# fmfi-compbio/warpstr

Measured on NVIDIA B200. Metric: caller_reads_per_s, higher is better.
Workload: dtype f64

## Files before the change

### warpstr_b200/csrc/dtw.cu

```cuda
#include "wstr_internal.h"

namespace {

constexpr int CH = WSTR_SIG_CHUNK;
constexpr unsigned FULL = 0xffffffffu;

__device__ __forceinline__ uint32_t smem_u32(const void *p) {
    return static_cast<uint32_t>(__cvta_generic_to_shared(p));
}
__device__ __forceinline__ void mbar_init(uint64_t *bar, int count) {
    asm volatile("mbarrier.init.shared::cta.b64 [%0], %1;" ::"r"(smem_u32(bar)), "r"(count) : "memory");
}
__device__ __forceinline__ void fence_barrier_init() {
    asm volatile("fence.mbarrier_init.release.cluster;" ::: "memory");
    asm volatile("fence.proxy.async.shared::cta;" ::: "memory");
}
__device__ __forceinline__ void bulk_load(void *dst, const void *src, uint32_t bytes, uint64_t *bar) {
    asm volatile("mbarrier.arrive.expect_tx.shared::cta.b64 _, [%0], %1;" ::"r"(smem_u32(bar)), "r"(bytes)
                 : "memory");
    asm volatile(
        "cp.async.bulk.shared::cluster.global.mbarrier::complete_tx::bytes [%0], [%1], %2, [%3];" ::"r"(
            smem_u32(dst)),
        "l"(src), "r"(bytes), "r"(smem_u32(bar))
        : "memory");
}
__device__ __forceinline__ bool mbar_try_wait(uint64_t *bar, uint32_t parity) {
    uint32_t ok;
    asm volatile(
        "{\n"
        ".reg .pred p;\n"
        "mbarrier.try_wait.parity.shared::cta.b64 p, [%1], %2;\n"
        "selp.u32 %0, 1, 0, p;\n"
        "}\n"
        : "=r"(ok)
        : "r"(smem_u32(bar)), "r"(parity)
        : "memory");
    return ok != 0;
}

__device__ __forceinline__ double dinf() { return __longlong_as_double(0x7ff0000000000000LL); }

template <int K, int MV>
struct LaneState {
    double v[K];
    double D[K];
    double R[MV - 1][K];
};

template <int MV>
__host__ __device__ constexpr int role_reg(int m, int ph) {
    return ((m - 1 - ph) % (MV - 1) + (MV - 1)) % (MV - 1);
}

template <int K, int MV, bool SHORT, int PH>
__device__ __forceinline__ double offer(const LaneState<K, MV> &s, int k) {
    if (SHORT) {
        if (MV >= 3) return s.R[role_reg<MV>(MV >= 3 ? MV - 2 : 1, PH)][k];
        return s.D[k];
    }
    return s.R[role_reg<MV>(MV - 1, PH)][k];
}

template <int K, int MV, int PH>
__device__ __forceinline__ void advance(LaneState<K, MV> &s, int k, double ae, double stay) {
#pragma unroll
    for (int m = MV - 2; m >= 1; --m) s.R[role_reg<MV>(m, PH)][k] += ae;
    s.R[role_reg<MV>(MV - 1, PH)][k] = stay;
}

template <int KG>
struct LaneConsts {
    uint32_t band_bits;
    uint32_t src0;
    uint32_t gsrc[KG];
};

template <int KG>
__host__ __device__ constexpr int q_row_len() { return 32 * KG + 40; }

template <int DEG>
struct DegOf {
    static constexpr bool LOW = DEG >= 100 && DEG < 200;
    static constexpr bool GRADED = DEG >= 200;
    static constexpr int MAX = GRADED ? (DEG - 200) / 10 : (LOW ? DEG - 100 : DEG);
};
template <int KG, int DEG>
__host__ __device__ constexpr int slot_deg(int g) {
    if (DegOf<DEG>::GRADED) return g == KG - 1 ? (DEG - 200) / 10 : (g == KG - 2 ? (DEG - 200) % 10 : 1);
    return (DegOf<DEG>::LOW && g < KG - 1) ? 1 : DegOf<DEG>::MAX;
}
template <int KC, int KG, int DEG>
__host__ __device__ constexpr int slot_bit(int g) {
    int b = KC;
    for (int i = 0; i < g; ++i) b += slot_deg<KG, DEG>(i);
    return b;
}
template <int KC, int KG, int DEG>
struct DirFmt {
    static constexpr int NB = slot_bit<KC, KG, DEG>(KG - 1) + DegOf<DEG>::MAX;
    static constexpr int RPW = 32 / NB;
    static_assert(NB <= 32 && RPW >= 1, "direction codes of one row must fit a 32-bit word");
};

struct DirOut {
    uint32_t acc;
    int sh;
    uint32_t *ptr;
};

__device__ __forceinline__ double take_min(const double best, uint32_t &codes, const double cand, const uint32_t bit) {
    double out;
    asm("{\n"
        ".reg .pred p;\n"
        "setp.lt.f64 p, %2, %3;\n"
        "selp.f64 %0, %2, %3, p;\n"
        "@p or.b32 %1, %1, %4;\n"
        "}\n"
        : "=d"(out), "+r"(codes)
        : "d"(cand), "d"(best), "r"(bit));
    return out;
}

template <int KC, int KG, int DEG, int MV, bool SHORT, bool BAND, int PH, int SUB>
__device__ __forceinline__ void dp_row(LaneState<KC + KG, MV> &s, const LaneConsts<KG> &lc, const double x,
                                       double *__restrict__ Qpub, const double *__restrict__ Qrow, DirOut &o) {
    constexpr int K = KC + KG;
    constexpr int NB = DirFmt<KC, KG, DEG>::NB, RPW = DirFmt<KC, KG, DEG>::RPW;
    constexpr int B0 = SUB >= 0 ? SUB * NB : 0;
    const double INF = dinf();

#pragma unroll
    for (int g = 0; g < KG; ++g) Qpub[g * 32] = offer<K, MV, SHORT, PH>(s, KC + g);
    Qpub[KG * 32] = offer<K, MV, SHORT, PH>(s, KC - 1);
    __syncwarp();

    uint32_t codes = SUB >= 0 ? o.acc : 0u;

    const double qfirst = *reinterpret_cast<const double *>(reinterpret_cast<const unsigned char *>(Qrow) + lc.src0);
#pragma unroll
    for (int k = KC - 1; k >= 0; --k) {
        const double ae = fabs(x - s.v[k]);
        const double qprev = k > 0 ? offer<K, MV, SHORT, PH>(s, k > 0 ? k - 1 : 0) : qfirst;
        const double stay = s.D[k] + ae;
        double best = stay;
        best = take_min(best, codes, qprev + ae, 1u << (B0 + k));
        if (BAND) {
            if ((lc.band_bits >> k) & 1u) {
                best = INF;
                codes &= ~(1u << (B0 + k));
            }
        }
        advance<K, MV, PH>(s, k, ae, stay);
        s.D[k] = best;
    }

#pragma unroll
    for (int g = 0; g < KG; ++g) {
        const int k = KC + g;
        const double ae = fabs(x - s.v[k]);
        const double stay = s.D[k] + ae;
        double best = stay;
#pragma unroll
        for (int r = 0; r < DegOf<DEG>::MAX; ++r) {
            if (r < slot_deg<KG, DEG>(g)) {
                const uint32_t idx = (lc.gsrc[g] >> (8 * r)) & 0xffu;
                best = take_min(best, codes, Qrow[idx] + ae, 1u << (B0 + slot_bit<KC, KG, DEG>(g) + r));
            }
        }
        if (BAND) {
            if ((lc.band_bits >> k) & 1u) {
                best = INF;
                codes &= ~(((1u << slot_deg<KG, DEG>(g)) - 1u) << (B0 + slot_bit<KC, KG, DEG>(g)));
            }
        }
        advance<K, MV, PH>(s, k, ae, stay);
        s.D[k] = best;
    }

    if (SUB >= 0) {
        if (SUB == RPW - 1) {
            *o.ptr = codes;
            o.ptr += 32;
            o.acc = 0u;
        } else {
            o.acc = codes;
        }
    } else {
        o.acc |= codes << o.sh;
        o.sh += NB;
        if (o.sh > 32 - NB) {
            *o.ptr = o.acc;
            o.ptr += 32;
            o.acc = 0u;
            o.sh = 0;
        }
    }
}

template <int KC, int KG, int DEG, int MV, bool SHORT, bool BAND, bool ALIGNED, int PH = 0>
__device__ __forceinline__ void dp_rows_cycle(LaneState<KC + KG, MV> &s, const LaneConsts<KG> &lc,
                                              double (&xv)[MV - 1], const double *__restrict__ xnext,
                                              double *__restrict__ Qlane, const double *__restrict__ Qbase,
                                              DirOut &o) {
    constexpr int QL = q_row_len<KG>();
    constexpr int RPW = DirFmt<KC, KG, DEG>::RPW;
    constexpr int SUB = RPW == 1 ? 0 : (ALIGNED ? PH : -1);
    dp_row<KC, KG, DEG, MV, SHORT, BAND, PH, SUB>(s, lc, xv[PH], Qlane + PH * QL, Qbase + PH * QL, o);
    xv[PH] = xnext[PH];
    if constexpr (PH + 1 < MV - 1)
        dp_rows_cycle<KC, KG, DEG, MV, SHORT, BAND, ALIGNED, PH + 1>(s, lc, xv, xnext, Qlane, Qbase, o);
}

template <int KC, int KG, int DEG, int MV, bool SHORT, bool BAND>
__device__ __forceinline__ void dp_row_single(LaneState<KC + KG, MV> &s, const LaneConsts<KG> &lc, const double x,
                                              double *__restrict__ Qlane, const double *__restrict__ Qbase,
                                              DirOut &o) {
    constexpr int K = KC + KG;
    constexpr int SUB = DirFmt<KC, KG, DEG>::RPW == 1 ? 0 : -1;
    dp_row<KC, KG, DEG, MV, SHORT, BAND, 0, SUB>(s, lc, x, Qlane, Qbase, o);
    __syncwarp();
#pragma unroll
    for (int k = 0; k < K; ++k) {
        const double last = s.R[MV - 2][k];
#pragma unroll
        for (int m = MV - 2; m >= 1; --m) s.R[m][k] = s.R[m - 1][k];
        s.R[0][k] = last;
    }
}

template <int KC, int KG, int DEG, int MV, bool SHORT, bool BAND>
__device__ __forceinline__ void dp_segment(LaneState<KC + KG, MV> &s, const LaneConsts<KG> &lc,
                                           const double *__restrict__ xs, const int tile0, int i0, const int i1,
                                           double *__restrict__ Qlane, const double *__restrict__ Qbase, DirOut &o) {
    constexpr int CY = MV - 1;
    constexpr int RPW = DirFmt<KC, KG, DEG>::RPW;
    constexpr bool ALIGNED = RPW == CY && RPW > 1;
    const double *xp = xs + (i0 - tile0);
    if (ALIGNED) {
#pragma unroll 1
        for (; i0 < i1 && o.sh != 0; ++i0) {
            dp_row_single<KC, KG, DEG, MV, SHORT, BAND>(s, lc, *xp, Qlane, Qbase, o);
            xp += 1;
        }
    }
    double xv[CY];
#pragma unroll
    for (int j = 0; j < CY; ++j) xv[j] = xp[j];
#pragma unroll 1
    for (; i0 + CY <= i1; i0 += CY) {
        dp_rows_cycle<KC, KG, DEG, MV, SHORT, BAND, ALIGNED>(s, lc, xv, xp + CY, Qlane, Qbase, o);
        xp += CY;
    }
#pragma unroll 1
    for (; i0 < i1; ++i0) {
        dp_row_single<KC, KG, DEG, MV, SHORT, BAND>(s, lc, *xp, Qlane, Qbase, o);
        xp += 1;
    }
}

__device__ __forceinline__ int mask_run_end(const uint32_t *__restrict__ mw, int a, const int limit, uint32_t &bit) {
    uint32_t word = __ldg(mw + (a >> 5));
    bit = (word >> (a & 31)) & 1u;
    uint32_t diff = (bit ? ~word : word) >> (a & 31);
    int b = a;
    for (;;) {
        if (diff) {
            b += __ffs(diff) - 1;
            break;
        }
        b = (b | 31) + 1;
        if (b >= limit) break;
        word = __ldg(mw + (b >> 5));
        diff = bit ? ~word : word;
    }
    return b < limit ? b : limit;
}

template <int KC, int KG, int DEG, int MV, bool BAND, bool MASKED>
__device__ __forceinline__ void dp_tile_rows(LaneState<KC + KG, MV> &s, const LaneConsts<KG> &lc,
                                             const double *__restrict__ xs, const int tile0, int i0, const int i1,
                                             const uint32_t *__restrict__ mw_ptr, double *__restrict__ Qlane,
                                             const double *__restrict__ Qbase, DirOut &o) {
    if (!MASKED || !mw_ptr) {
        dp_segment<KC, KG, DEG, MV, false, BAND>(s, lc, xs, tile0, i0, i1, Qlane, Qbase, o);
        return;
    }
    while (i0 < i1) {
        uint32_t bit;
        const int b = mask_run_end(mw_ptr, i0, i1, bit);
        if (bit) dp_segment<KC, KG, DEG, MV, true, BAND>(s, lc, xs, tile0, i0, b, Qlane, Qbase, o);
        else dp_segment<KC, KG, DEG, MV, false, BAND>(s, lc, xs, tile0, i0, b, Qlane, Qbase, o);
        i0 = b;
    }
}

template <int RPW>
struct TbGeom {
    static constexpr int WRW = RPW == 1 ? 16 : 32 / RPW;
    static constexpr int ROWS = WRW * RPW;
    static constexpr int NBUF = 5;
    static constexpr int WORDS = NBUF * WRW * 32;
};

__device__ __forceinline__ void mbar_expect_tx(uint64_t *bar, uint32_t bytes) {
    asm volatile("mbarrier.arrive.expect_tx.shared::cta.b64 _, [%0], %1;" ::"r"(smem_u32(bar)), "r"(bytes)
                 : "memory");
}
template <int KC, int KG, int DEG>
__device__ __forceinline__ void traceback_warp(const DevAutomaton *A, const int T, const uint32_t *dir,
                                               const uint32_t *mw, int32_t *tr, int32_t *status_slot,
                                               const int lane, uint32_t *win, uint64_t *bar, uint32_t &phase_bits,
                                               const int32_t *spred) {
    constexpr int K = KC + KG;
    constexpr int NB = DirFmt<KC, KG, DEG>::NB, RPW = DirFmt<KC, KG, DEG>::RPW;
    using G = TbGeom<RPW>;
    constexpr int WRW = G::WRW, ROWS = G::ROWS, NBUF = G::NBUF;
    const int mv = A->mv;
    const int wtop = (T - 1) / RPW;
    const int wmin = mv / RPW;
    const int nwin = wtop / WRW + 1;

    auto issue = [&](int c) {
        if (lane != 0) return;
        const int b = c % NBUF;
        const int wh = wtop - c * WRW;
        const int wfirst = wh - WRW + 1;
        const int w0 = wfirst > wmin ? wfirst : wmin;
        const int n = wh - w0 + 1;
        if (n > 0)
            bulk_load(win + (b * WRW + (w0 - wfirst)) * 32, dir + static_cast<int64_t>(w0) * 32,
                      static_cast<uint32_t>(n) * 128u, &bar[b]);
        else
            mbar_expect_tx(&bar[b], 0u);
    };

    int i = T - 1;
    int pos = A->end_pos;
    int st = __ldg(A->state_of_pos + pos);
    bool failed = false;
    for (int c = 0; c < nwin && c < NBUF; ++c) issue(c);

    for (int c = 0; c < nwin; ++c) {
        const int b = c % NBUF;
        while (!mbar_try_wait(&bar[b], (phase_bits >> b) & 1u)) {
        }
        phase_bits ^= 1u << b;
        const int wh = wtop - c * WRW;
        const int hi = wh * RPW + RPW - 1;
        const int lo = hi - ROWS + 1 > 0 ? hi - ROWS + 1 : 0;
        if (i >= lo && i > 0 && !failed) {
            const int row = hi - lane;
            const bool mine = lane < ROWS && row >= lo && row <= i;
            const bool coded = mine && row >= mv;
            uint32_t mb = 0u;
            if (mw && mine) mb = (__ldg(mw + (row >> 5)) >> (row & 31)) & 1u;
            const int wr = mine ? row / RPW : wh;
            const uint32_t *wslot = win + (b * WRW + (wr - (wh - WRW + 1))) * 32;
            const int fsh = (row - wr * RPW) * NB;
            int my = st;
            for (;;) {
                const int hl = pos / K;
                const int u = pos - hl * K;
                uint32_t nib = 0u;
                if (coded && row <= i) {
                    const uint32_t f = wslot[hl] >> fsh;
                    if (u < KC) {
                        nib = (f >> u) & 1u;
                    } else {
                        const int g = u - KC;
                        int off = KC, width = 1;
#pragma unroll
                        for (int gg = 0; gg < KG; ++gg)
                            if (g == gg) {
                                off = slot_bit<KC, KG, DEG>(gg);
                                width = slot_deg<KG, DEG>(gg);
                            }
                        nib = (f >> off) & ((1u << width) - 1u);
                    }
                }
                const uint32_t moves = __ballot_sync(FULL, nib != 0u);
                if (moves == 0u) {
                    i = lo - 1;
                    break;
                }
                const int tm = __ffs(moves) - 1;
                const int rm = hi - tm;
                const uint32_t nibm = __shfl_sync(FULL, nib, tm);
                const int back = mv - static_cast<int>(__shfl_sync(FULL, mb, tm));
                const int code = 31 - __clz(nibm);
                const int32_t pp = spred[pos * DegOf<DEG>::MAX + code];
                if (rm < back || pp < 0) {
                    failed = true;
                    break;
                }
                const int pst = pp >> 16;
                if (row < rm) my = pst;
                if (rm - back + 1 < lo) {
                    const int r = lo - 1 - lane;
                    if (lane < back - 1 && r > rm - back) tr[r] = pst;
                }
                i = rm - back;
                pos = pp & 0xffff;
                st = pst;
                if (i < lo || i <= 0) break;
            }
            if (mine) tr[row] = my;
        }
        __syncwarp();
        if (c + NBUF < nwin) issue(c + NBUF);
    }
    if (lane == 0) {
        if (failed) *status_slot = WSTR_READ_BACKTRACK;
        else tr[0] = st;
    }
}

template <int KC, int KG, int DEG, int MV>
struct alignas(16) FillSmem {
    using G = TbGeom<DirFmt<KC, KG, DEG>::RPW>;
    double sig[2][CH];
    double Q[MV - 1][q_row_len<KG>()];
    uint32_t win[G::WORDS];
    int32_t pred[(KC + KG) * 32 * DegOf<DEG>::MAX];
    uint64_t bar[2];
    uint64_t tbar[G::NBUF];
};

#ifndef WSTR_K8_WARPS
#define WSTR_K8_WARPS 16
#endif
#ifdef WSTR_MAXNREG
#define WSTR_FILL_BOUNDS __maxnreg__(WSTR_MAXNREG)
#else
#define WSTR_FILL_BOUNDS                         \
    __launch_bounds__(32 * WSTR_WARPS_PER_CTA,   \
                      ((KC + KG) * (MV + 1) <= 45 && KG <= 1 && !MASKED ? WSTR_K8_WARPS                                          \
                       : ((KC + KG) * (MV + 1) <= 60 && KC + KG <= 12 ? 12 : 8)) / WSTR_WARPS_PER_CTA)
#endif
template <int KC, int KG, int DEG, int MV, bool MASKED>
__global__ void WSTR_FILL_BOUNDS dtw_fill_kernel(const FillParams p) {
    extern __shared__ __align__(16) unsigned char smem_raw[];
    constexpr int K = KC + KG;
    constexpr int NB = DirFmt<KC, KG, DEG>::NB, RPW = DirFmt<KC, KG, DEG>::RPW;
    const int warp = WSTR_WARPS_PER_CTA == 1 ? 0 : static_cast<int>(threadIdx.x >> 5);
    const int lane = WSTR_WARPS_PER_CTA == 1 ? static_cast<int>(threadIdx.x) : static_cast<int>(threadIdx.x & 31);
    using Smem = FillSmem<KC, KG, DEG, MV>;
    Smem &sm = reinterpret_cast<Smem *>(smem_raw)[warp];
    const double INF = dinf();

    if (lane == 0) {
        mbar_init(&sm.bar[0], 1);
        mbar_init(&sm.bar[1], 1);
        for (int b = 0; b < Smem::G::NBUF; ++b) mbar_init(&sm.tbar[b], 1);
        fence_barrier_init();
    }
    for (int e = lane; e < (MV - 1) * q_row_len<KG>(); e += 32) (&sm.Q[0][0])[e] = INF;
    __syncwarp();
    uint32_t uses0 = 0, uses1 = 0;
    uint32_t tb_phase = 0;

    LaneState<K, MV> s;
    LaneConsts<KG> lc;
    int cached_aut = -1;
    double v0 = 0.0;

    for (int taken = 0; taken < p.n; ++taken) {
        int r = 0;
        if (lane == 0) r = atomicAdd(p.queue, 1);
        r = __shfl_sync(FULL, r, 0);
        if (r >= p.n) break;
        const ReadMeta m = p.meta[p.order[r]];
        const DevAutomaton *A = p.auts + m.aut;
        const int T = m.T;
        if (p.respect_status && p.status[m.read] != WSTR_READ_OK) continue;
        if (T <= MV) {
            if (lane == 0) p.status[m.read] = WSTR_READ_TOO_SHORT;
            continue;
        }

        if (m.aut != cached_aut) {
#pragma unroll
            for (int k = 0; k < K; ++k) s.v[k] = __ldg(A->v_pos + lane * K + k);
            lc.band_bits = __ldg(A->lane_tab + lane * WSTR_LANE_TAB_STRIDE + 0);
            lc.src0 = __ldg(A->lane_tab + lane * WSTR_LANE_TAB_STRIDE + 1) * 8u;
#pragma unroll
            for (int g = 0; g < KG; ++g) lc.gsrc[g] = __ldg(A->lane_tab + lane * WSTR_LANE_TAB_STRIDE + 2 + g);
            v0 = __ldg(A->v_pos + A->init_pos[0]);
            constexpr int DM = DegOf<DEG>::MAX;
            for (int e = lane; e < K * 32 * DM; e += 32)
                sm.pred[e] = __ldg(A->pred_tab + (e / DM) * WSTR_PRED_STRIDE + 1 + (e % DM));
            cached_aut = m.aut;
        }

        const double *gsig = p.signal + m.sig_off;
        const int nchunks = (T + CH - 1) / CH;
        auto issue = [&](int c) {
            if (lane == 0) {
                int n = T - c * CH;
                n = n > CH ? CH : n;
                n = (n + 1) & ~1;
                bulk_load(sm.sig[c & 1], gsig + static_cast<int64_t>(c) * CH, static_cast<uint32_t>(n) * 8u,
                          &sm.bar[c & 1]);
            }
        };
        issue(0);
        if (nchunks > 1) issue(1);
        while (!mbar_try_wait(&sm.bar[0], uses0 & 1u)) {
        }
        ++uses0;

        {
            const double *x0 = sm.sig[0];
            const double first = fabs(x0[0] - v0);
#pragma unroll
            for (int k = 0; k < K; ++k) {
                s.D[k] = INF;
#pragma unroll
                for (int mm = 0; mm < MV - 1; ++mm) s.R[mm][k] = INF;
            }
            for (int c = 0; c <= MV; ++c) {
                const int pos = A->init_pos[c];
                double d0 = first;
                if (c > 0) d0 = first + fabs(x0[c] - v0);
#pragma unroll
                for (int k = 0; k < K; ++k) {
                    if (pos == lane * K + k) {
                        double acc = d0;
                        for (int t = 1; t <= MV - 1; ++t) acc = acc + fabs(x0[t] - s.v[k]);
                        s.R[MV - 2][k] = acc;
                    }
                }
            }
        }

        const int band_start = max(A->th1, T - A->band6 + 1);
        const int band_free = A->band_closed ? band_start + MV : T;
        const uint32_t *mw_ptr = MASKED && p.maskbits ? p.maskbits + m.mask_off : nullptr;
        uint32_t *dir = p.dir + m.dir_off;
        DirOut o;
        o.acc = 0u;
        o.sh = (MV % RPW) * NB;
        o.ptr = dir + (MV / RPW) * 32 + lane;
        double *Qlane = &sm.Q[0][0] + lane;
        const double *Qbase = &sm.Q[0][0];

        for (int c = 0; c < nchunks; ++c) {
            if (c > 0) {
                if (c & 1) {
                    while (!mbar_try_wait(&sm.bar[1], uses1 & 1u)) {
                    }
                    ++uses1;
                } else {
                    while (!mbar_try_wait(&sm.bar[0], uses0 & 1u)) {
                    }
                    ++uses0;
                }
            }
            const double *xs = sm.sig[c & 1];
            const int i_begin = c == 0 ? MV : c * CH;
            const int i_end = min(T, (c + 1) * CH);
            for (int a = i_begin; a < i_end;) {
                const bool banded = a >= band_start && a < band_free;
                const int e = banded ? min(i_end, band_free) : (a < band_start ? min(i_end, band_start) : i_end);
                if (banded) dp_tile_rows<KC, KG, DEG, MV, true, MASKED>(s, lc, xs, c * CH, a, e, mw_ptr, Qlane, Qbase, o);
                else dp_tile_rows<KC, KG, DEG, MV, false, MASKED>(s, lc, xs, c * CH, a, e, mw_ptr, Qlane, Qbase, o);
                a = e;
            }
            __syncwarp();
            if (c + 2 < nchunks) issue(c + 2);
        }

        if (o.sh != 0) *o.ptr = o.acc;
        if (p.end_cost) {
            const int ep = A->end_pos;
#pragma unroll
            for (int k = 0; k < K; ++k)
                if (ep == lane * K + k) p.end_cost[m.read] = s.D[k];
        }
        if (lane == 0) p.status[m.read] = WSTR_READ_OK;
        __syncwarp();
#ifndef WSTR_NO_TRACEBACK
        traceback_warp<KC, KG, DEG>(A, T, dir, mw_ptr, p.trace + m.sig_off, p.status + m.read, lane, sm.win, sm.tbar,
                                    tb_phase, sm.pred);
#endif
    }
}

template <int KC, int KG, int DEG, int MV, bool MASKED>
int launch_fill_m(const FillParams &p, cudaStream_t s) {
    static int grid_cap = 0;
    static unsigned long long attr_done = 0ull;
    const int smem = static_cast<int>(sizeof(FillSmem<KC, KG, DEG, MV>)) * WSTR_WARPS_PER_CTA;
    int dev = 0;
    WSTR_CUDA(cudaGetDevice(&dev));
    if (grid_cap == 0 || !((attr_done >> (dev & 63)) & 1ull)) {
        WSTR_CUDA(cudaFuncSetAttribute(dtw_fill_kernel<KC, KG, DEG, MV, MASKED>,
                                       cudaFuncAttributeMaxDynamicSharedMemorySize, smem));
        WSTR_CUDA(cudaFuncSetAttribute(dtw_fill_kernel<KC, KG, DEG, MV, MASKED>,
                                       cudaFuncAttributePreferredSharedMemoryCarveout,
                                       cudaSharedmemCarveoutMaxShared));
        int sms = 0, per_sm = 0;
        WSTR_CUDA(cudaDeviceGetAttribute(&sms, cudaDevAttrMultiProcessorCount, dev));
        WSTR_CUDA(cudaOccupancyMaxActiveBlocksPerMultiprocessor(&per_sm, dtw_fill_kernel<KC, KG, DEG, MV, MASKED>,
                                                                32 * WSTR_WARPS_PER_CTA, smem));
        if (per_sm < 1) per_sm = 1;
        grid_cap = sms * per_sm;
        attr_done |= 1ull << (dev & 63);
    }
    int grid = (p.n + WSTR_WARPS_PER_CTA - 1) / WSTR_WARPS_PER_CTA;
    if (grid > grid_cap) grid = grid_cap;
    if (grid < 1) return WSTR_OK;
    dtw_fill_kernel<KC, KG, DEG, MV, MASKED><<<grid, 32 * WSTR_WARPS_PER_CTA, smem, s>>>(p);
    WSTR_CUDA(cudaGetLastError());
    return WSTR_OK;
}

template <int KC, int KG, int DEG, int MV>
int launch_fill_t(const FillParams &p, cudaStream_t s) {
    if (p.maskbits) return launch_fill_m<KC, KG, DEG, MV, true>(p, s);
    return launch_fill_m<KC, KG, DEG, MV, false>(p, s);
}

template <int KC, int KG, int MV>
int launch_fill_deg(int deg, const FillParams &p, cudaStream_t s) {
    if (deg == 2) return launch_fill_t<KC, KG, 2, MV>(p, s);
    if (deg == 4) return launch_fill_t<KC, KG, 4, MV>(p, s);
    if constexpr (KG >= 2 && MV == 4) {
        if (deg == 102) return launch_fill_t<KC, KG, 102, MV>(p, s);
        if (deg == 104) return launch_fill_t<KC, KG, 104, MV>(p, s);
    }
    if constexpr (KG >= 3 && MV == 4) {
        if (deg == 242) return launch_fill_t<KC, KG, 242, MV>(p, s);
    }
    return WSTR_ERR_UNSUPPORTED;
}

}

#ifdef WSTR_FILL_PART
#define WSTR_HAS_PART(n) (WSTR_FILL_PART == (n))
#else
#define WSTR_HAS_PART(n) 1
#endif
#define WSTR_CASE(KC_, KG_, MV_) \
    if (kc == KC_ && kg == KG_ && mv == MV_) return launch_fill_deg<KC_, KG_, MV_>(deg, p, s);

#define WSTR_DECL_PART(n) int wstr_launch_fill_p##n(int kc, int kg, int deg, int mv, const FillParams &p, cudaStream_t s);
WSTR_DECL_PART(0)
WSTR_DECL_PART(1)
WSTR_DECL_PART(2)
WSTR_DECL_PART(3)
WSTR_DECL_PART(4)
WSTR_DECL_PART(5)
WSTR_DECL_PART(6)
WSTR_DECL_PART(7)
WSTR_DECL_PART(8)
#undef WSTR_DECL_PART

#if WSTR_HAS_PART(0)
int wstr_launch_fill_p0(int kc, int kg, int deg, int mv, const FillParams &p, cudaStream_t s) {
    WSTR_CASE(7, 1, 4)
    WSTR_CASE(8, 1, 4)
    WSTR_CASE(6, 2, 2)
    WSTR_CASE(6, 2, 3)
    return WSTR_ERR_UNSUPPORTED;
}

int wstr_launch_fill(int kc, int kg, int deg, int mv, const FillParams &p, cudaStream_t s) {
    typedef int (*part_fn)(int, int, int, int, const FillParams &, cudaStream_t);
    static const part_fn parts[] = {wstr_launch_fill_p0, wstr_launch_fill_p1, wstr_launch_fill_p2,
                                    wstr_launch_fill_p3, wstr_launch_fill_p4, wstr_launch_fill_p5,
                                    wstr_launch_fill_p6, wstr_launch_fill_p7, wstr_launch_fill_p8};
    for (part_fn f : parts) {
        const int rc = f(kc, kg, deg, mv, p, s);
        if (rc != WSTR_ERR_UNSUPPORTED) return rc;
    }
    return WSTR_ERR_UNSUPPORTED;
}
#endif
#if WSTR_HAS_PART(1)
int wstr_launch_fill_p1(int kc, int kg, int deg, int mv, const FillParams &p, cudaStream_t s) {
    WSTR_CASE(6, 2, 4)
    WSTR_CASE(6, 2, 5)
    WSTR_CASE(6, 2, 6)
    return WSTR_ERR_UNSUPPORTED;
}
#endif
#if WSTR_HAS_PART(2)
int wstr_launch_fill_p2(int kc, int kg, int deg, int mv, const FillParams &p, cudaStream_t s) {
    WSTR_CASE(4, 4, 4)
    WSTR_CASE(8, 2, 4)
    WSTR_CASE(6, 4, 4)
    return WSTR_ERR_UNSUPPORTED;
}
#endif
#if WSTR_HAS_PART(3)
int wstr_launch_fill_p3(int kc, int kg, int deg, int mv, const FillParams &p, cudaStream_t s) {
    WSTR_CASE(8, 4, 4)
    WSTR_CASE(12, 4, 4)
    return WSTR_ERR_UNSUPPORTED;
}
#endif
#if WSTR_HAS_PART(4)
int wstr_launch_fill_p4(int kc, int kg, int deg, int mv, const FillParams &p, cudaStream_t s) {
    WSTR_CASE(6, 4, 2)
    WSTR_CASE(6, 4, 3)
    return WSTR_ERR_UNSUPPORTED;
}
#endif
#if WSTR_HAS_PART(5)
int wstr_launch_fill_p5(int kc, int kg, int deg, int mv, const FillParams &p, cudaStream_t s) {
    WSTR_CASE(6, 4, 5)
    WSTR_CASE(6, 4, 6)
    return WSTR_ERR_UNSUPPORTED;
}
#endif
#if WSTR_HAS_PART(6)
int wstr_launch_fill_p6(int kc, int kg, int deg, int mv, const FillParams &p, cudaStream_t s) {
    WSTR_CASE(7, 2, 4)
    WSTR_CASE(7, 4, 4)
    return WSTR_ERR_UNSUPPORTED;
}
#endif
#if WSTR_HAS_PART(7)
int wstr_launch_fill_p7(int kc, int kg, int deg, int mv, const FillParams &p, cudaStream_t s) {
    WSTR_CASE(6, 2, 7)
    WSTR_CASE(6, 2, 8)
    return WSTR_ERR_UNSUPPORTED;
}
#endif
#if WSTR_HAS_PART(8)
int wstr_launch_fill_p8(int kc, int kg, int deg, int mv, const FillParams &p, cudaStream_t s) {
    WSTR_CASE(6, 4, 7)
    WSTR_CASE(6, 4, 8)
    return WSTR_ERR_UNSUPPORTED;
}
#endif
#undef WSTR_CASE
```

Baseline: 1.064 million.

## Batch tracebacks per lane across 32 reads with register prefetch ring

Replaces the warp-cooperative traceback, which used TMA-loaded direction windows, ballots and shuffles, with a per-lane scalar traceback. Each warp queues up to 32 finished reads and then traces them in parallel, one read per lane. Each lane keeps a small register ring of prefetched direction words and writes state runs directly. Predecessor tables are now read from global memory instead of shared memory, which shrinks the shared-memory footprint and may allow higher occupancy. The trade-off is serial dependent-load chains and divergence between lanes whose reads differ in length.

```diff
diff --git a/warpstr_b200/csrc/dtw.cu b/warpstr_b200/csrc/dtw.cu
--- a/warpstr_b200/csrc/dtw.cu
+++ b/warpstr_b200/csrc/dtw.cu
@@ -294,136 +294,135 @@
     }
 }
 
-template <int RPW>
-struct TbGeom {
-    static constexpr int WRW = RPW == 1 ? 16 : 32 / RPW;
-    static constexpr int ROWS = WRW * RPW;
-    static constexpr int NBUF = 5;
-    static constexpr int WORDS = NBUF * WRW * 32;
-};
-
-__device__ __forceinline__ void mbar_expect_tx(uint64_t *bar, uint32_t bytes) {
-    asm volatile("mbarrier.arrive.expect_tx.shared::cta.b64 _, [%0], %1;" ::"r"(smem_u32(bar)), "r"(bytes)
-                 : "memory");
-}
+#ifndef WSTR_TB_AHEAD
+#define WSTR_TB_AHEAD 8
+#endif
+constexpr int TB_AHEAD = WSTR_TB_AHEAD;
+
+template <int NB, int RPW>
+__host__ __device__ constexpr uint32_t row_rep() {
+    uint32_t r = 0u;
+    for (int s = 0; s < RPW; ++s) r |= 1u << (s * NB);
+    return r;
+}
+
 template <int KC, int KG, int DEG>
-__device__ __forceinline__ void traceback_warp(const DevAutomaton *A, const int T, const uint32_t *dir,
-                                               const uint32_t *mw, int32_t *tr, int32_t *status_slot,
-                                               const int lane, uint32_t *win, uint64_t *bar, uint32_t &phase_bits,
-                                               const int32_t *spred) {
+__device__ __forceinline__ void slot_field(const int u, int &off, uint32_t &wmask) {
+    off = u;
+    wmask = 1u;
+    if (u >= KC) {
+#pragma unroll
+        for (int g = 0; g < KG; ++g)
+            if (u - KC == g) {
+                off = slot_bit<KC, KG, DEG>(g);
+                wmask = (1u << slot_deg<KG, DEG>(g)) - 1u;
+            }
+    }
+}
+
+__device__ __forceinline__ void put_run(int32_t *tr, const int a, int b, const int32_t state) {
+#ifdef WSTR_TB_ST2
+    if (b >= a && !(b & 1)) tr[b--] = state;
+    for (; b - 1 >= a; b -= 2) *reinterpret_cast<int2 *>(tr + b - 1) = make_int2(state, state);
+    if (b == a) tr[b] = state;
+#else
+    for (; b >= a; --b) tr[b] = state;
+#endif
+}
+
+template <int KC, int KG, int DEG, int MV, bool MASKED>
+__device__ __forceinline__ void traceback_lane(const FillParams &p, const ReadMeta &m) {
     constexpr int K = KC + KG;
     constexpr int NB = DirFmt<KC, KG, DEG>::NB, RPW = DirFmt<KC, KG, DEG>::RPW;
-    using G = TbGeom<RPW>;
-    constexpr int WRW = G::WRW, ROWS = G::ROWS, NBUF = G::NBUF;
-    const int mv = A->mv;
-    const int wtop = (T - 1) / RPW;
-    const int wmin = mv / RPW;
-    const int nwin = wtop / WRW + 1;
-
-    auto issue = [&](int c) {
-        if (lane != 0) return;
-        const int b = c % NBUF;
-        const int wh = wtop - c * WRW;
-        const int wfirst = wh - WRW + 1;
-        const int w0 = wfirst > wmin ? wfirst : wmin;
-        const int n = wh - w0 + 1;
-        if (n > 0)
-            bulk_load(win + (b * WRW + (w0 - wfirst)) * 32, dir + static_cast<int64_t>(w0) * 32,
-                      static_cast<uint32_t>(n) * 128u, &bar[b]);
-        else
-            mbar_expect_tx(&bar[b], 0u);
-    };
-
-    int i = T - 1;
+    constexpr int PF = TB_AHEAD;
+    constexpr int WMIN = MV / RPW;
+    constexpr uint32_t REP = row_rep<NB, RPW>();
+    const DevAutomaton *A = p.auts + m.aut;
+    const uint32_t *dir = p.dir + m.dir_off;
+    const uint32_t *mw = MASKED && p.maskbits ? p.maskbits + m.mask_off : nullptr;
+    const int32_t *pred = A->pred_tab;
+    int32_t *tr = p.trace + m.sig_off;
+
+    int i = m.T - 1;
     int pos = A->end_pos;
-    int st = __ldg(A->state_of_pos + pos);
+    int32_t st = __ldg(A->state_of_pos + pos);
+    int hl = pos / K;
+    int off;
+    uint32_t wmask;
+    slot_field<KC, KG, DEG>(pos - hl * K, off, wmask);
+    uint32_t fm = (wmask << off) * REP;
+    const uint32_t *col = dir + hl;
+    auto fetch = [&](const int w) -> uint32_t { return w >= WMIN ? col[static_cast<int64_t>(w) * 32] : 0u; };
+
+    int W = i / RPW;
+    uint32_t wb[PF];
+#pragma unroll
+    for (int k = 0; k < PF; ++k) wb[k] = fetch(W - k);
     bool failed = false;
-    for (int c = 0; c < nwin && c < NBUF; ++c) issue(c);
-
-    for (int c = 0; c < nwin; ++c) {
-        const int b = c % NBUF;
-        while (!mbar_try_wait(&bar[b], (phase_bits >> b) & 1u)) {
-        }
-        phase_bits ^= 1u << b;
-        const int wh = wtop - c * WRW;
-        const int hi = wh * RPW + RPW - 1;
-        const int lo = hi - ROWS + 1 > 0 ? hi - ROWS + 1 : 0;
-        if (i >= lo && i > 0 && !failed) {
-            const int row = hi - lane;
-            const bool mine = lane < ROWS && row >= lo && row <= i;
-            const bool coded = mine && row >= mv;
-            uint32_t mb = 0u;
-            if (mw && mine) mb = (__ldg(mw + (row >> 5)) >> (row & 31)) & 1u;
-            const int wr = mine ? row / RPW : wh;
-            const uint32_t *wslot = win + (b * WRW + (wr - (wh - WRW + 1))) * 32;
-            const int fsh = (row - wr * RPW) * NB;
-            int my = st;
+    while (i >= MV) {
+#pragma unroll
+        for (int j = 0; j < PF; ++j) {
             for (;;) {
-                const int hl = pos / K;
-                const int u = pos - hl * K;
-                uint32_t nib = 0u;
-                if (coded && row <= i) {
-                    const uint32_t f = wslot[hl] >> fsh;
-                    if (u < KC) {
-                        nib = (f >> u) & 1u;
-                    } else {
-                        const int g = u - KC;
-                        int off = KC, width = 1;
-#pragma unroll
-                        for (int gg = 0; gg < KG; ++gg)
-                            if (g == gg) {
-                                off = slot_bit<KC, KG, DEG>(gg);
-                                width = slot_deg<KG, DEG>(gg);
-                            }
-                        nib = (f >> off) & ((1u << width) - 1u);
-                    }
-                }
-                const uint32_t moves = __ballot_sync(FULL, nib != 0u);
-                if (moves == 0u) {
-                    i = lo - 1;
+                const int sub = i - W * RPW;
+                if (i < MV || sub < 0) break;
+                const uint32_t hit = wb[j] & fm & (0xffffffffu >> (32 - (sub + 1) * NB));
+                if (hit == 0u) {
+                    put_run(tr, W * RPW, i, st);
+                    i = W * RPW - 1;
                     break;
                 }
-                const int tm = __ffs(moves) - 1;
-                const int rm = hi - tm;
-                const uint32_t nibm = __shfl_sync(FULL, nib, tm);
-                const int back = mv - static_cast<int>(__shfl_sync(FULL, mb, tm));
-                const int code = 31 - __clz(nibm);
-                const int32_t pp = spred[pos * DegOf<DEG>::MAX + code];
+                const int s = (31 - __clz(hit)) / NB;
+                const int rm = W * RPW + s;
+                const uint32_t code = (wb[j] >> (s * NB + off)) & wmask;
+                const int back = MV - (mw ? static_cast<int>((__ldg(mw + (rm >> 5)) >> (rm & 31)) & 1u) : 0);
+                const int32_t pp = __ldg(pred + pos * WSTR_PRED_STRIDE + 1 + (31 - __clz(code)));
                 if (rm < back || pp < 0) {
                     failed = true;
+                    i = -1;
                     break;
                 }
-                const int pst = pp >> 16;
-                if (row < rm) my = pst;
-                if (rm - back + 1 < lo) {
-                    const int r = lo - 1 - lane;
-                    if (lane < back - 1 && r > rm - back) tr[r] = pst;
-                }
+                put_run(tr, rm, i, st);
+                st = pp >> 16;
+                put_run(tr, rm - back + 1, rm - 1, st);
                 i = rm - back;
                 pos = pp & 0xffff;
-                st = pst;
-                if (i < lo || i <= 0) break;
-            }
-            if (mine) tr[row] = my;
-        }
-        __syncwarp();
-        if (c + NBUF < nwin) issue(c + NBUF);
-    }
-    if (lane == 0) {
-        if (failed) *status_slot = WSTR_READ_BACKTRACK;
-        else tr[0] = st;
-    }
+                const int nhl = pos / K;
+                slot_field<KC, KG, DEG>(pos - nhl * K, off, wmask);
+                fm = (wmask << off) * REP;
+                if (nhl != hl) {
+                    hl = nhl;
+                    col = dir + hl;
+#pragma unroll
+                    for (int k = 0; k < PF; ++k) wb[(j + k) % PF] = fetch(W - k);
+                }
+            }
+            if (i < MV) break;
+#ifdef WSTR_TB_PFL1
+            if (W - 2 * PF >= WMIN) asm volatile("prefetch.global.L1 [%0];" ::"l"(col + static_cast<int64_t>(W - 2 * PF) * 32));
+#endif
+            wb[j] = fetch(W - PF);
+            --W;
+        }
+    }
+    if (failed) p.status[m.read] = WSTR_READ_BACKTRACK;
+    else put_run(tr, 0, i, st);
+}
+
+template <int KC, int KG, int DEG, int MV, bool MASKED, class Smem>
+__device__ __forceinline__ void traceback_batch(const FillParams &p, Smem &sm, const int lane) {
+    if (lane < sm.tbn) traceback_lane<KC, KG, DEG, MV, MASKED>(p, p.meta[sm.tbq[lane]]);
+    __syncwarp();
+    if (lane == 0) sm.tbn = 0;
+    __syncwarp();
 }
 
 template <int KC, int KG, int DEG, int MV>
 struct alignas(16) FillSmem {
-    using G = TbGeom<DirFmt<KC, KG, DEG>::RPW>;
     double sig[2][CH];
     double Q[MV - 1][q_row_len<KG>()];
-    uint32_t win[G::WORDS];
-    int32_t pred[(KC + KG) * 32 * DegOf<DEG>::MAX];
     uint64_t bar[2];
-    uint64_t tbar[G::NBUF];
+    int32_t tbq[32];
+    int32_t tbn;
 };
 
 #ifndef WSTR_K8_WARPS
@@ -451,13 +450,12 @@
     if (lane == 0) {
         mbar_init(&sm.bar[0], 1);
         mbar_init(&sm.bar[1], 1);
-        for (int b = 0; b < Smem::G::NBUF; ++b) mbar_init(&sm.tbar[b], 1);
         fence_barrier_init();
+        sm.tbn = 0;
     }
     for (int e = lane; e < (MV - 1) * q_row_len<KG>(); e += 32) (&sm.Q[0][0])[e] = INF;
     __syncwarp();
     uint32_t uses0 = 0, uses1 = 0;
-    uint32_t tb_phase = 0;
 
     LaneState<K, MV> s;
     LaneConsts<KG> lc;
@@ -470,6 +468,7 @@
         r = __shfl_sync(FULL, r, 0);
         if (r >= p.n) break;
         const ReadMeta m = p.meta[p.order[r]];
+        if (lane == 0) sm.tbq[sm.tbn] = p.order[r];
         const DevAutomaton *A = p.auts + m.aut;
         const int T = m.T;
         if (p.respect_status && p.status[m.read] != WSTR_READ_OK) continue;
@@ -486,9 +485,6 @@
 #pragma unroll
             for (int g = 0; g < KG; ++g) lc.gsrc[g] = __ldg(A->lane_tab + lane * WSTR_LANE_TAB_STRIDE + 2 + g);
             v0 = __ldg(A->v_pos + A->init_pos[0]);
-            constexpr int DM = DegOf<DEG>::MAX;
-            for (int e = lane; e < K * 32 * DM; e += 32)
-                sm.pred[e] = __ldg(A->pred_tab + (e / DM) * WSTR_PRED_STRIDE + 1 + (e % DM));
             cached_aut = m.aut;
         }
 
@@ -578,12 +574,16 @@
                 if (ep == lane * K + k) p.end_cost[m.read] = s.D[k];
         }
         if (lane == 0) p.status[m.read] = WSTR_READ_OK;
+#ifndef WSTR_NO_TRACEBACK
+        if (lane == 0) ++sm.tbn;
         __syncwarp();
+        if (sm.tbn == 32) traceback_batch<KC, KG, DEG, MV, MASKED>(p, sm, lane);
+#endif
+    }
 #ifndef WSTR_NO_TRACEBACK
-        traceback_warp<KC, KG, DEG>(A, T, dir, mw_ptr, p.trace + m.sig_off, p.status + m.read, lane, sm.win, sm.tbar,
-                                    tb_phase, sm.pred);
-#endif
-    }
+    __syncwarp();
+    if (sm.tbn > 0) traceback_batch<KC, KG, DEG, MV, MASKED>(p, sm, lane);
+#endif
 }
 
 template <int KC, int KG, int DEG, int MV, bool MASKED>
@@ -598,7 +598,11 @@
                                        cudaFuncAttributeMaxDynamicSharedMemorySize, smem));
         WSTR_CUDA(cudaFuncSetAttribute(dtw_fill_kernel<KC, KG, DEG, MV, MASKED>,
                                        cudaFuncAttributePreferredSharedMemoryCarveout,
+#ifdef WSTR_TB_CARVE
+                                       WSTR_TB_CARVE));
+#else
                                        cudaSharedmemCarveoutMaxShared));
+#endif
         int sms = 0, per_sm = 0;
         WSTR_CUDA(cudaDeviceGetAttribute(&sms, cudaDevAttrMultiProcessorCount, dev));
         WSTR_CUDA(cudaOccupancyMaxActiveBlocksPerMultiprocessor(&per_sm, dtw_fill_kernel<KC, KG, DEG, MV, MASKED>,
```

After: 667,400, median of 6. 37.3% lower.
